# zfwangDP/X2-GNN

Measured on AMD Instinct MI355X. Metric: molecules/sec (fwd+bwd) on QM9 U0, batch=128, 1/2/4/8 MI355X, higher is better.
Workload: dtype fp32; 1 GPU; xgnn_poly U0 train step (config.json: L=4, D=128, H=16, sbf 7x6), S160, fwd+loss+bwd+allreduce+clip+Adam+EMA; per_gpu_batch=128, global_batch=128, line_nodes_per_gpu=21058, triplets_per_gpu=194060, parallelism=dp1, hip_graph=True

## Files before the change

x2-gnn_amd/csrc/feature.hip:

```cpp
#include "common.hpp"

namespace x2g {
namespace {

typedef float f4 __attribute__((ext_vector_type(4)));

constexpr int kFN1 = 256;
constexpr int kFN2 = 128;
constexpr int kFKMax = 384;
constexpr int kFRows = 32;
constexpr int kFAS = kFKMax + 8;
constexpr int kFYS = kFN1 + 8;
constexpr int kFThreads = 512;

__device__ __forceinline__ f4 mfma4(float a, float b, f4 acc) {
  return __builtin_amdgcn_mfma_f32_16x16x4f32(a, b, acc, 0, 0, 0);
}
__device__ __forceinline__ float sigmoid_(float z) {
  return __builtin_amdgcn_rcpf(1.0f + __builtin_amdgcn_exp2f(-1.4426950408889634f * z));
}
__device__ __forceinline__ float silu_(float z) { return z * sigmoid_(z); }
__device__ __forceinline__ float silu_grad_(float z) {
  const float s = sigmoid_(z);
  return s * (1.0f + z * (1.0f - s));
}
__device__ __forceinline__ f4 zero4() { return f4{0.f, 0.f, 0.f, 0.f}; }

__device__ __forceinline__ f4 quad_t(f4 v, int j) {
  f4 b, c;
#pragma unroll
  for (int k = 0; k < 4; ++k) {
    const float t = dpp_mov<0xB1>(v[k ^ 1]);
    b[k] = ((k ^ j) & 1) ? t : v[k];
  }
#pragma unroll
  for (int k = 0; k < 4; ++k) {
    const float t = dpp_mov<0x4E>(b[k ^ 2]);
    c[k] = ((k ^ j) & 2) ? t : b[k];
  }
  return c;
}

__device__ __forceinline__ int64_t tpos(int64_t tf, int64_t tile16, int f, int g) {
  return (f >> 7) * tf + tile16 * 2048 + (f & 127) * 16 + 4 * g;
}

struct FeatFwdArgs {
  const float* x;
  const float* env;
  const float* w1;
  const float* b1;
  const float* w2;
  const float* b2;
  float* y2;
  float* xs_t;
  float* z1_t;
  float* y1_t;
  float* z2_t;
  int64_t R;
  int64_t tf;
  int K;
  int want_t;
};

__device__ __forceinline__ f4 w1_frag(const float* __restrict__ w1, int K, int c, int q, int g) {
  const int k = 16 * q + 4 * g;
  const int k0 = k < K ? k : K - 2, k1 = k + 2 < K ? k + 2 : K - 2;
  const float2 lo = *reinterpret_cast<const float2*>(w1 + c * K + k0);
  const float2 hi = *reinterpret_cast<const float2*>(w1 + c * K + k1);
  const float m0 = k < K ? 1.0f : 0.0f, m1 = k + 2 < K ? 1.0f : 0.0f;
  return f4{lo.x * m0, lo.y * m0, hi.x * m1, hi.y * m1};
}

constexpr int kFX4 = (kFRows * kFKMax / 4 + kFThreads - 1) / kFThreads;

struct XTile {
  f4 v[kFX4];
  float env;
};

__device__ __forceinline__ void xtile_load(const FeatFwdArgs& a, int64_t tile, XTile& t) {
  const int64_t r0 = tile * kFRows;
  const int64_t R = a.R;
  const int nr = R - r0 < kFRows ? static_cast<int>(R - r0) : kFRows;
  const float* src = a.x + r0 * a.K;
  const int n = nr * a.K;
#pragma unroll
  for (int u = 0; u < kFX4; ++u) {
    const int q = threadIdx.x + kFThreads * u;
    if (4 * q + 3 < n) {
      t.v[u] = *reinterpret_cast<const f4*>(src + 4 * q);
    } else {
#pragma unroll
      for (int e = 0; e < 4; ++e) t.v[u][e] = 4 * q + e < n ? src[4 * q + e] : 0.0f;
    }
  }
  const int r = threadIdx.x;
  t.env = (r < nr && a.env) ? a.env[r0 + r] : 1.0f;
}

__global__ void __launch_bounds__(kFThreads, 1) feat_fwd_kernel(const FeatFwdArgs a) {
  __shared__ __attribute__((aligned(16))) float A[kFRows * kFAS];
  __shared__ __attribute__((aligned(16))) float Y1[kFRows * kFYS];
  __shared__ float envs[kFRows];
  const int tid = threadIdx.x, lane = tid & 63, w = tid >> 6;
  const int i = lane & 15, g = lane >> 4;
  const int K = a.K, KQ = (K + 15) / 16;
  const float invK = 1.0f / static_cast<float>(K);
  const int64_t R = a.R;
  const float* w2s = a.w2 + (16 * w + i) * kFN1 + 4 * g;
  const float b2v = a.b2 ? a.b2[16 * w + i] : 0.0f;
  const int c1a = 32 * w + i, c1b = c1a + 16;
  const float b1a = a.b1 ? a.b1[c1a] : 0.0f, b1b = a.b1 ? a.b1[c1b] : 0.0f;
  for (int idx = tid; idx < kFRows * (kFKMax - K); idx += kFThreads) {
    const int r = idx / (kFKMax - K), c = K + idx % (kFKMax - K);
    A[r * kFAS + c] = 0.0f;
  }
  const int64_t ntiles = (R + kFRows - 1) / kFRows;
  XTile xt;
  if (static_cast<int64_t>(blockIdx.x) < ntiles) xtile_load(a, blockIdx.x, xt);
  for (int64_t tile = blockIdx.x; tile < ntiles; tile += gridDim.x) {
    const int64_t r0 = tile * kFRows;
    const int nr = R - r0 < kFRows ? static_cast<int>(R - r0) : kFRows;
    __syncthreads();
    {
      const int n = nr * K;
#pragma unroll
      for (int u = 0; u < kFX4; ++u) {
        const int q = tid + kFThreads * u;
#pragma unroll
        for (int e = 0; e < 4; ++e) {
          const int j = 4 * q + e;
          if (j < kFRows * K) {
            int r = static_cast<int>(static_cast<float>(j) * invK);
            r -= r * K > j ? 1 : 0;
            r += (r + 1) * K <= j ? 1 : 0;
            A[r * kFAS + (j - r * K)] = j < n ? xt.v[u][e] : 0.0f;
          }
        }
      }
      if (tid < kFRows) envs[tid] = xt.env;
    }
    __syncthreads();
    f4 wa0 = w1_frag(a.w1, K, c1a, 0, g), wb0 = w1_frag(a.w1, K, c1b, 0, g);
    f4 wa1 = w1_frag(a.w1, K, c1a, 1, g), wb1 = w1_frag(a.w1, K, c1b, 1, g);
    if (tile + gridDim.x < ntiles) xtile_load(a, tile + gridDim.x, xt);
    auto xs_store = [&](int it) {
      const int rt = it / 3, p = it % 3;
      const int64_t t16 = r0 / 16 + rt;
      if (!a.want_t || t16 * 16 >= R || 128 * p >= K) return;
      const int f = tid >> 2, rr = 16 * rt + 4 * (tid & 3);
      f4 v;
#pragma unroll
      for (int e = 0; e < 4; ++e) v[e] = A[(rr + e) * kFAS + 128 * p + f] * envs[rr + e];
      *reinterpret_cast<f4*>(a.xs_t + p * a.tf + t16 * 2048 + 4 * tid) = v;
    };
    f4 acc[2][2] = {{zero4(), zero4()}, {zero4(), zero4()}};
    const int KQn = KQ;
    f4 a0 = *reinterpret_cast<const f4*>(A + i * kFAS + 4 * g);
    f4 a1 = *reinterpret_cast<const f4*>(A + (16 + i) * kFAS + 4 * g);
    auto group = [&](int q, f4& ba, f4& bb) {
      const int qa = q + 1 < KQn ? q + 1 : q;
      const f4 n0 = *reinterpret_cast<const f4*>(A + i * kFAS + 16 * qa + 4 * g);
      const f4 n1 = *reinterpret_cast<const f4*>(A + (16 + i) * kFAS + 16 * qa + 4 * g);
#pragma unroll
      for (int e = 0; e < 4; ++e) {
        acc[0][0] = mfma4(a0[e], ba[e], acc[0][0]);
        acc[0][1] = mfma4(a0[e], bb[e], acc[0][1]);
        acc[1][0] = mfma4(a1[e], ba[e], acc[1][0]);
        acc[1][1] = mfma4(a1[e], bb[e], acc[1][1]);
      }
      const int qb = q + 2 < KQn ? q + 2 : q;
      ba = w1_frag(a.w1, K, c1a, qb, g);
      bb = w1_frag(a.w1, K, c1b, qb, g);
      a0 = n0;
      a1 = n1;
    };
    for (int q = 0; q < KQn; q += 2) {
      group(q, wa0, wb0);
      if (q + 1 < KQn) group(q + 1, wa1, wb1);
    }
    f4 wq[3];
    wq[0] = *reinterpret_cast<const f4*>(w2s);
    wq[1] = *reinterpret_cast<const f4*>(w2s + 16);
#pragma unroll
    for (int rb = 0; rb < 2; ++rb) {
      const int64_t t16 = r0 / 16 + rb;
      const bool tile_ok = t16 * 16 < R;
#pragma unroll
      for (int cb = 0; cb < 2; ++cb) {
        const int c = cb ? c1b : c1a;
        const float bias = cb ? b1b : b1a;
        f4 z, y;
#pragma unroll
        for (int e = 0; e < 4; ++e) {
          const int r = 16 * rb + 4 * g + e;
          const bool ok = r < nr;
          z[e] = ok ? fmaf(acc[rb][cb][e], envs[r], bias) : 0.0f;
          y[e] = ok ? silu_(z[e]) : 0.0f;
          Y1[r * kFYS + c] = y[e];
        }
        if (tile_ok && a.want_t) {
          *reinterpret_cast<f4*>(a.z1_t + tpos(a.tf, t16, c, g)) = z;
          *reinterpret_cast<f4*>(a.y1_t + tpos(a.tf, t16, c, g)) = y;
        }
      }
    }
    __syncthreads();
    f4 acc2[2] = {zero4(), zero4()};
    {
      f4 y0 = *reinterpret_cast<const f4*>(Y1 + i * kFYS + 4 * g);
      f4 y1 = *reinterpret_cast<const f4*>(Y1 + (16 + i) * kFYS + 4 * g);
#pragma unroll
      for (int q = 0; q < 16; ++q) {
        const int qa = q + 1 < 16 ? q + 1 : q;
        const f4 n0 = *reinterpret_cast<const f4*>(Y1 + i * kFYS + 16 * qa + 4 * g);
        const f4 n1 = *reinterpret_cast<const f4*>(Y1 + (16 + i) * kFYS + 16 * qa + 4 * g);
        if (q + 2 < 16) wq[(q + 2) % 3] = *reinterpret_cast<const f4*>(w2s + 16 * (q + 2));
        __builtin_amdgcn_sched_barrier(0);
#pragma unroll
        for (int e = 0; e < 4; ++e) {
          acc2[0] = mfma4(y0[e], wq[q % 3][e], acc2[0]);
          acc2[1] = mfma4(y1[e], wq[q % 3][e], acc2[1]);
        }
        y0 = n0;
        y1 = n1;
      }
    }
    const int c2 = 16 * w + i;
    const int qj = i & 3, qm = i >> 2;
#pragma unroll
    for (int rb = 0; rb < 2; ++rb) {
      const int64_t t16 = r0 / 16 + rb;
      if (t16 * 16 >= R) continue;
      f4 z, y;
#pragma unroll
      for (int e = 0; e < 4; ++e) {
        const int r = 16 * rb + 4 * g + e;
        z[e] = r < nr ? acc2[rb][e] + b2v : 0.0f;
        y[e] = silu_(z[e]);
      }
      const f4 yt = quad_t(y, qj);
      const int ry = 16 * rb + 4 * g + qj;
      if (ry < nr) *reinterpret_cast<f4*>(a.y2 + (r0 + ry) * kFN2 + 16 * w + 4 * qm) = yt;
      if (a.want_t) *reinterpret_cast<f4*>(a.z2_t + tpos(a.tf, t16, c2, g)) = z;
    }
    for (int it = 0; it < 6; ++it) xs_store(it);
  }
}

struct FeatBwdArgs {
  const float* dy;
  const float* z2_t;
  const float* z1_t;
  const float* w2;
  float* dz2_t;
  float* dz1_t;
  int64_t R;
  int64_t tf;
};

constexpr int kFDS = kFN2 + 8;

__global__ void __launch_bounds__(kFThreads, 1) feat_bwd_kernel(const FeatBwdArgs a) {
  __shared__ __attribute__((aligned(16))) float DZ[kFRows * kFDS];
  const int tid = threadIdx.x, lane = tid & 63, w = tid >> 6;
  const int i = lane & 15, g = lane >> 4;
  const int64_t R = a.R;
  const int ca = 32 * w + i, cb = ca + 16;
  f4 wa[8], wb[8];
#pragma unroll
  for (int q = 0; q < 8; ++q)
#pragma unroll
    for (int e = 0; e < 4; ++e) {
      wa[q][e] = a.w2[(16 * q + 4 * g + e) * kFN1 + ca];
      wb[q][e] = a.w2[(16 * q + 4 * g + e) * kFN1 + cb];
    }
  const int c2 = 16 * w + i;
  const int64_t ntiles = (R + kFRows - 1) / kFRows;
  struct In {
    f4 z2[2];
    float dy[2][4];
  };
  auto load_in = [&](int64_t tile, In& in) {
    const int64_t r0 = tile * kFRows;
    const int nr = R - r0 < kFRows ? static_cast<int>(R - r0) : kFRows;
#pragma unroll
    for (int rb = 0; rb < 2; ++rb) {
      const int64_t t16 = r0 / 16 + rb;
      in.z2[rb] = t16 * 16 < R ? *reinterpret_cast<const f4*>(a.z2_t + tpos(a.tf, t16, c2, g)) : zero4();
#pragma unroll
      for (int e = 0; e < 4; ++e) {
        const int r = 16 * rb + 4 * g + e;
        in.dy[rb][e] = r < nr ? a.dy[(r0 + r) * kFN2 + c2] : 0.0f;
      }
    }
  };
  In cur;
  if (static_cast<int64_t>(blockIdx.x) < ntiles) load_in(blockIdx.x, cur);
  for (int64_t tile = blockIdx.x; tile < ntiles; tile += gridDim.x) {
    const int64_t r0 = tile * kFRows;
    const int nr = R - r0 < kFRows ? static_cast<int>(R - r0) : kFRows;
    __syncthreads();
#pragma unroll
    for (int rb = 0; rb < 2; ++rb) {
      const int64_t t16 = r0 / 16 + rb;
      const bool tile_ok = t16 * 16 < R;
      f4 d;
#pragma unroll
      for (int e = 0; e < 4; ++e) {
        const int r = 16 * rb + 4 * g + e;
        d[e] = r < nr ? cur.dy[rb][e] * silu_grad_(cur.z2[rb][e]) : 0.0f;
        DZ[r * kFDS + c2] = d[e];
      }
      if (tile_ok) *reinterpret_cast<f4*>(a.dz2_t + tpos(a.tf, t16, c2, g)) = d;
    }
    f4 z1v[2][2];
#pragma unroll
    for (int rb = 0; rb < 2; ++rb) {
      const int64_t t16 = r0 / 16 + rb;
      const int64_t tt = t16 * 16 < R ? t16 : r0 / 16;
#pragma unroll
      for (int k = 0; k < 2; ++k) z1v[rb][k] = *reinterpret_cast<const f4*>(a.z1_t + tpos(a.tf, tt, k ? cb : ca, g));
    }
    if (tile + gridDim.x < ntiles) load_in(tile + gridDim.x, cur);
    __syncthreads();
    f4 acc[2][2] = {{zero4(), zero4()}, {zero4(), zero4()}};
#pragma unroll
    for (int q = 0; q < 8; ++q) {
      const f4 a0 = *reinterpret_cast<const f4*>(DZ + i * kFDS + 16 * q + 4 * g);
      const f4 a1 = *reinterpret_cast<const f4*>(DZ + (16 + i) * kFDS + 16 * q + 4 * g);
#pragma unroll
      for (int e = 0; e < 4; ++e) {
        acc[0][0] = mfma4(a0[e], wa[q][e], acc[0][0]);
        acc[0][1] = mfma4(a0[e], wb[q][e], acc[0][1]);
        acc[1][0] = mfma4(a1[e], wa[q][e], acc[1][0]);
        acc[1][1] = mfma4(a1[e], wb[q][e], acc[1][1]);
      }
    }
#pragma unroll
    for (int rb = 0; rb < 2; ++rb) {
      const int64_t t16 = r0 / 16 + rb;
      if (t16 * 16 >= R) continue;
#pragma unroll
      for (int k = 0; k < 2; ++k) {
        const int c = k ? cb : ca;
        f4 d;
#pragma unroll
        for (int e = 0; e < 4; ++e) d[e] = acc[rb][k][e] * silu_grad_(z1v[rb][k][e]);
        *reinterpret_cast<f4*>(a.dz1_t + tpos(a.tf, t16, c, g)) = d;
      }
    }
  }
}

inline bool al16(const void* p) { return reinterpret_cast<uintptr_t>(p) % 16 == 0; }

inline unsigned feat_grid(int64_t R) {
  const int64_t tiles = (R + kFRows - 1) / kFRows;
  return static_cast<unsigned>(tiles < 256 ? tiles : 256);
}

}
}

using namespace x2g;

X2G_API int x2g_feat_fwd(const float* x, const float* env, int64_t rows, int32_t in_dim, const float* w1,
                         const float* b1, const float* w2, const float* b2, float* y, float* xs_t, float* z1_t,
                         float* y1_t, float* z2_t, void* stream) {
  if (rows < 0 || in_dim <= 0) return X2G_EINVAL;
  if (in_dim > kFKMax || in_dim % 2 || in_dim <= 2 * 128 || rows * kFKMax * 4 >= (int64_t(1) << 31))
    return X2G_EUNSUPPORTED;
  if (rows == 0) return X2G_OK;
  if (!x || !w1 || !w2 || !y) return X2G_EINVAL;
  const int nt = (xs_t != nullptr) + (z1_t != nullptr) + (y1_t != nullptr) + (z2_t != nullptr);
  if (nt != 0 && nt != 4) return X2G_EINVAL;
  if (!al16(x) || !al16(w2) || !al16(xs_t) || !al16(z1_t) || !al16(y1_t) || !al16(z2_t) ||
      reinterpret_cast<uintptr_t>(w1) % 8)
    return X2G_EUNSUPPORTED;
  FeatFwdArgs a{x, env, w1, b1, w2, b2, y, xs_t, z1_t, y1_t, z2_t, rows, x2g_chain_t_floats(rows, 128), in_dim,
                nt == 4 ? 1 : 0};
  feat_fwd_kernel<<<feat_grid(rows), kFThreads, 0, as_stream(stream)>>>(a);
  return last_launch_status();
}

X2G_API int x2g_feat_bwd(const float* dy, const float* z2_t, const float* z1_t, const float* w2, int64_t rows,
                         float* dz2_t, float* dz1_t, void* stream) {
  if (rows < 0) return X2G_EINVAL;
  if (rows * kFKMax * 4 >= (int64_t(1) << 31)) return X2G_EUNSUPPORTED;
  if (rows == 0) return X2G_OK;
  if (!dy || !z2_t || !z1_t || !w2 || !dz2_t || !dz1_t) return X2G_EINVAL;
  if (!al16(z2_t) || !al16(z1_t) || !al16(dz2_t) || !al16(dz1_t)) return X2G_EUNSUPPORTED;
  FeatBwdArgs a{dy, z2_t, z1_t, w2, dz2_t, dz1_t, rows, x2g_chain_t_floats(rows, 128)};
  feat_bwd_kernel<<<feat_grid(rows), kFThreads, 0, as_stream(stream)>>>(a);
  return last_launch_status();
}
```

x2-gnn_amd/csrc/rbf_gate.hip:

```cpp
#include "common.hpp"

namespace x2g {

constexpr int kGateRMax = 8;
constexpr int kGateBwdSplits = 128;

typedef float f4v __attribute__((ext_vector_type(4)));

template <int D>
__device__ __forceinline__ void stage_gate_weights(const float* __restrict__ W, const float* __restrict__ B, int R,
                                                   float* __restrict__ sw) {
  for (int i = threadIdx.x; i < D * R; i += blockDim.x) sw[i] = W[i];
  for (int i = threadIdx.x; i < D; i += blockDim.x) sw[D * kGateRMax + i] = B ? B[i] : 0.f;
  __syncthreads();
}

template <int LPR>
struct GateW {
  float w[4][kGateRMax];
  float b[4];
  __device__ __forceinline__ void load(const float* __restrict__ sw, int R, int sub) {
    constexpr int D = 4 * LPR;
#pragma unroll
    for (int i = 0; i < 4; ++i) {
      const int c = 4 * sub + i;
#pragma unroll
      for (int j = 0; j < kGateRMax; ++j) w[i][j] = j < R ? sw[c * R + j] : 0.f;
      b[i] = sw[D * kGateRMax + c];
    }
  }
  __device__ __forceinline__ f4v filter(const float (&rb)[kGateRMax]) const {
    f4v f;
#pragma unroll
    for (int i = 0; i < 4; ++i) {
      float a = b[i];
#pragma unroll
      for (int j = 0; j < kGateRMax; ++j) a = fmaf(w[i][j], rb[j], a);
      f[i] = a;
    }
    return f;
  }
};

__device__ __forceinline__ void load_rbf(const float* __restrict__ rbf, int64_t r, int R, float (&rb)[kGateRMax]) {
#pragma unroll
  for (int j = 0; j < kGateRMax; ++j) rb[j] = rbf[r * R + (j < R ? j : R - 1)];
}

template <int LPR>
__global__ void __launch_bounds__(256) rbf_gate_fwd_kernel(const f4v* __restrict__ x, const float* __restrict__ rbf,
                                                           const float* __restrict__ W, const float* __restrict__ B,
                                                           int64_t rows, int R, f4v* __restrict__ out) {
  constexpr int RPB = 256 / LPR;
  constexpr int UNROLL = 4;
  __shared__ float sw[4 * LPR * (kGateRMax + 1)];
  stage_gate_weights<4 * LPR>(W, B, R, sw);
  const int sub = threadIdx.x % LPR, slot = threadIdx.x / LPR;
  GateW<LPR> gw;
  gw.load(sw, R, sub);
  const int64_t stride = static_cast<int64_t>(gridDim.x) * RPB * UNROLL;
  for (int64_t r0 = static_cast<int64_t>(blockIdx.x) * RPB * UNROLL + slot; r0 < rows; r0 += stride) {
    float rb[UNROLL][kGateRMax];
    f4v xv[UNROLL];
#pragma unroll
    for (int u = 0; u < UNROLL; ++u) {
      const int64_t r = r0 + u * RPB, rc = r < rows ? r : rows - 1;
      load_rbf(rbf, rc, R, rb[u]);
      xv[u] = x[rc * LPR + sub];
    }
#pragma unroll
    for (int u = 0; u < UNROLL; ++u) {
      const int64_t r = r0 + u * RPB;
      if (r < rows) out[r * LPR + sub] = xv[u] * gw.filter(rb[u]);
    }
  }
}

constexpr int kGateMaxJobs = X2G_GATE_MAX_JOBS;
struct PoolJobs {
  const f4v* x[kGateMaxJobs];
  const float* w[kGateMaxJobs];
  const float* b[kGateMaxJobs];
  f4v* out[kGateMaxJobs];
};

template <int LPR>
__global__ void __launch_bounds__(256) rbf_pool_fwd_kernel(const PoolJobs J, const float* __restrict__ rbf,
                                                           const int32_t* __restrict__ rowptr, int64_t G, int R) {
  constexpr int RPI = 64 / LPR;
  constexpr int UNROLL = 8;
  __shared__ float sw[4 * LPR * (kGateRMax + 1)];
  const int job = blockIdx.y;
  const f4v* __restrict__ x = J.x[job];
  f4v* __restrict__ out = J.out[job];
  stage_gate_weights<4 * LPR>(J.w[job], J.b[job], R, sw);
  const int lane = threadIdx.x & 63;
  const int sub = lane % LPR, slot = lane / LPR;
  GateW<LPR> gw;
  gw.load(sw, R, sub);
  const int nwaves = gridDim.x * 4;
  const int jl = (lane & 15) < R ? (lane & 15) : R - 1;
  for (int64_t g = uniform(blockIdx.x * 4 + (threadIdx.x >> 6)); g < G; g += nwaves) {
    const int r0 = uniform(rowptr[g]), r1 = uniform(rowptr[g + 1]);
    f4v acc = {0.f, 0.f, 0.f, 0.f};
    for (int rb0 = r0; rb0 < r1; rb0 += UNROLL * RPI) {
      f4v v[UNROLL];
      float rv[UNROLL];
#pragma unroll
      for (int u = 0; u < UNROLL; ++u) {
        const int r = rb0 + u * RPI + slot;
        const int rc = r < r1 ? r : r1 - 1;
        v[u] = x[static_cast<int64_t>(rc) * LPR + sub];
        rv[u] = rbf[static_cast<int64_t>(rc) * R + jl];
      }
#pragma unroll
      for (int u = 0; u < UNROLL; ++u) {
        const float ok = rb0 + u * RPI + slot < r1 ? 1.f : 0.f;
        float rb[kGateRMax];
        rb[0] = dpp_mov<0x150>(rv[u]);
        rb[1] = dpp_mov<0x151>(rv[u]);
        rb[2] = dpp_mov<0x152>(rv[u]);
        rb[3] = dpp_mov<0x153>(rv[u]);
        rb[4] = dpp_mov<0x154>(rv[u]);
        rb[5] = dpp_mov<0x155>(rv[u]);
        rb[6] = dpp_mov<0x156>(rv[u]);
        rb[7] = dpp_mov<0x157>(rv[u]);
        acc += (v[u] * gw.filter(rb)) * ok;
      }
    }
#pragma unroll
    for (int off = LPR; off < 64; off <<= 1) {
#pragma unroll
      for (int i = 0; i < 4; ++i) acc[i] += __shfl_xor(acc[i], off, kWave);
    }
    if (slot == 0) out[g * LPR + sub] = acc;
  }
}

template <int LPR>
__device__ __forceinline__ float transpose_sum(const float (&p)[kGateRMax], int sub, int& j) {
  constexpr int o1 = LPR / 2, o2 = LPR / 4, o3 = LPR / 8;
  const bool h1 = sub & o1, h2 = sub & o2, h3 = sub & o3;
  float q[4], r[2];
#pragma unroll
  for (int k = 0; k < 4; ++k) {
    const float send = h1 ? p[k] : p[k + 4];
    const float recv = xor_xchg<o1>(send);
    q[k] = (h1 ? p[k + 4] : p[k]) + recv;
  }
#pragma unroll
  for (int k = 0; k < 2; ++k) {
    const float send = h2 ? q[k] : q[k + 2];
    const float recv = xor_xchg<o2>(send);
    r[k] = (h2 ? q[k + 2] : q[k]) + recv;
  }
  float t;
  {
    const float send = h3 ? r[0] : r[1];
    const float recv = xor_xchg<o3>(send);
    t = (h3 ? r[1] : r[0]) + recv;
  }
  if constexpr (o3 >= 8) t += xor_xchg<4>(t);
  if constexpr (o3 >= 4) t += xor_xchg<2>(t);
  if constexpr (o3 >= 2) t += xor_xchg<1>(t);
  j = 4 * h1 + 2 * h2 + h3;
  return t;
}

struct GateBwdJobs {
  const f4v* g[kGateMaxJobs];
  const f4v* x[kGateMaxJobs];
  const float* w[kGateMaxJobs];
  const float* b[kGateMaxJobs];
  f4v* dx[kGateMaxJobs];
  const f4v* dx_add[kGateMaxJobs];
  float* drbf[kGateMaxJobs];
  float* part_w[kGateMaxJobs];
  float* part_b[kGateMaxJobs];
};

template <int LPR>
__global__ void __launch_bounds__(256) rbf_gate_bwd_kernel(const GateBwdJobs J, const int32_t* __restrict__ owner,
                                                           const float* __restrict__ rbf, int64_t rows, int R,
                                                           int drbf_acc) {
  constexpr int RPB = 256 / LPR;
  constexpr int D = 4 * LPR;
  __shared__ float red[RPB * D * (kGateRMax + 1)];
  __shared__ float sw[D * (kGateRMax + 1)];
  const int job = blockIdx.y;
  const f4v* __restrict__ g = J.g[job];
  const f4v* __restrict__ x = J.x[job];
  f4v* __restrict__ dx = J.dx[job];
  const f4v* __restrict__ dx_add = J.dx_add[job];
  float* __restrict__ drbf = J.drbf[job];
  float* __restrict__ part_w = J.part_w[job];
  float* __restrict__ part_b = J.part_b[job];
  stage_gate_weights<D>(J.w[job], J.b[job], R, sw);
  const int sub = threadIdx.x % LPR, slot = threadIdx.x / LPR;
  GateW<LPR> gw;
  gw.load(sw, R, sub);
  float aw[4][kGateRMax], ab[4];
#pragma unroll
  for (int i = 0; i < 4; ++i) {
    ab[i] = 0.f;
#pragma unroll
    for (int j = 0; j < kGateRMax; ++j) aw[i][j] = 0.f;
  }
  constexpr int UNROLL = 3;
  const int jd = 4 * ((sub & (LPR / 2)) != 0) + 2 * ((sub & (LPR / 4)) != 0) + ((sub & (LPR / 8)) != 0);
  const bool acc_drbf = drbf && drbf_acc && jd < R;
  const int64_t per = (rows + gridDim.x - 1) / gridDim.x;
  const int64_t lo = per * blockIdx.x, hi = lo + per < rows ? lo + per : rows;
  const int jl = (threadIdx.x & 15) < R ? (threadIdx.x & 15) : R - 1;
  auto desc = [](const void* p, int64_t bytes) {
    return __builtin_amdgcn_make_buffer_rsrc(const_cast<void*>(p), static_cast<short>(0),
                                             static_cast<int>(bytes < 0x7fffffff ? bytes : 0x7fffffff), 0x00020000);
  };
  const __amdgpu_buffer_rsrc_t own_r = desc(owner, owner ? rows * 4 : 0);
  const __amdgpu_buffer_rsrc_t od_r = desc(drbf, (drbf && drbf_acc) ? rows * R * 4 : 0);
  const __amdgpu_buffer_rsrc_t add_r = desc(dx_add, dx_add ? rows * LPR * 16 : 0);
  const bool has_owner = owner != nullptr;
  for (int64_t r0 = lo + slot; r0 < hi; r0 += RPB * UNROLL) {
    float rv[UNROLL];
    f4v gv[UNROLL], xv[UNROLL], av[UNROLL];
    float od[UNROLL];
#pragma unroll
    for (int u = 0; u < UNROLL; ++u) {
      const int64_t r = r0 + u * RPB, rc = r < hi ? r : hi - 1;
      rv[u] = rbf[rc * R + jl];
      od[u] = __builtin_bit_cast(float, __builtin_amdgcn_raw_buffer_load_b32(
                                            od_r, acc_drbf ? static_cast<int>((rc * R + jd) * 4) : 0x7ffffff0, 0, 0));
      const int ow = static_cast<int>(__builtin_amdgcn_raw_buffer_load_b32(own_r, static_cast<int>(rc * 4), 0, 0));
      const int64_t o = has_owner ? ow : rc;
      gv[u] = g[o * LPR + sub];
      xv[u] = x[rc * LPR + sub];
      av[u] = __builtin_bit_cast(f4v, __builtin_amdgcn_raw_buffer_load_b128(
                                         add_r, static_cast<int>((rc * LPR + sub) * 16), 0, 0));
    }
#pragma unroll
    for (int u = 0; u < UNROLL; ++u) {
      const int64_t r = r0 + u * RPB;
      const bool ok = r < hi;
      const float m = ok ? 1.f : 0.f;
      float rb[kGateRMax];
      rb[0] = dpp_mov<0x150>(rv[u]);
      rb[1] = dpp_mov<0x151>(rv[u]);
      rb[2] = dpp_mov<0x152>(rv[u]);
      rb[3] = dpp_mov<0x153>(rv[u]);
      rb[4] = dpp_mov<0x154>(rv[u]);
      rb[5] = dpp_mov<0x155>(rv[u]);
      rb[6] = dpp_mov<0x156>(rv[u]);
      rb[7] = dpp_mov<0x157>(rv[u]);
      if (dx && ok) {
        f4v d = gv[u] * gw.filter(rb);
        if (dx_add) d += av[u];
        dx[r * LPR + sub] = d;
      }
      const f4v df = gv[u] * xv[u] * m;
#pragma unroll
      for (int i = 0; i < 4; ++i) {
        ab[i] += df[i];
#pragma unroll
        for (int j = 0; j < kGateRMax; ++j) aw[i][j] = fmaf(df[i], rb[j], aw[i][j]);
      }
      if (drbf) {
        float p[kGateRMax];
#pragma unroll
        for (int j = 0; j < kGateRMax; ++j) {
          float a = 0.f;
#pragma unroll
          for (int i = 0; i < 4; ++i) a = fmaf(df[i], gw.w[i][j], a);
          p[j] = a;
        }
        int j;
        const float tot = transpose_sum<LPR>(p, sub, j);
        if ((sub & (LPR / 8 - 1)) == 0 && ok && j < R) drbf[r * R + j] = tot + od[u];
      }
    }
  }
  const int per_slot = D * (R + 1);
  float* mine = red + slot * per_slot;
#pragma unroll
  for (int i = 0; i < 4; ++i) {
    const int c = 4 * sub + i;
    for (int j = 0; j < R; ++j) mine[c * R + j] = aw[i][j];
    mine[D * R + c] = ab[i];
  }
  __syncthreads();
  for (int idx = threadIdx.x; idx < per_slot; idx += 256) {
    float s = 0.f;
    for (int sl = 0; sl < RPB; ++sl) s += red[sl * per_slot + idx];
    if (idx < D * R)
      part_w[static_cast<int64_t>(blockIdx.x) * D * R + idx] = s;
    else if (part_b)
      part_b[static_cast<int64_t>(blockIdx.x) * D + idx - D * R] = s;
  }
}

inline bool gate_shape_ok(int D, int R) { return R >= 1 && R <= kGateRMax && (D == 64 || D == 128 || D == 256); }

inline int gate_bwd_splits(int64_t rows) {
  const int64_t want = (rows + 7) / 8;
  return static_cast<int>(want < kGateBwdSplits ? (want < 1 ? 1 : want) : kGateBwdSplits);
}

}

using namespace x2g;

static inline bool al16(const void* p) { return reinterpret_cast<uintptr_t>(p) % 16 == 0; }

X2G_API int x2g_rbf_gate_fwd(const float* x, const float* rbf, const float* w, const float* b, int64_t rows, int32_t D,
                             int32_t R, float* out, void* stream) {
  if (rows < 0 || !gate_shape_ok(D, R)) return rows < 0 ? X2G_EINVAL : X2G_EUNSUPPORTED;
  if (rows == 0) return X2G_OK;
  if (!x || !rbf || !w || !out) return X2G_EINVAL;
  if (!al16(x) || !al16(out)) return X2G_EINVAL;
  const auto* xv = reinterpret_cast<const f4v*>(x);
  auto* ov = reinterpret_cast<f4v*>(out);
  const int64_t want = (rows * D / 4 + 1023) / 1024;
  const unsigned grid = static_cast<unsigned>(want < 2048 ? want : 2048);
  hipStream_t st = as_stream(stream);
  switch (D) {
    case 64: rbf_gate_fwd_kernel<16><<<grid, 256, 0, st>>>(xv, rbf, w, b, rows, R, ov); break;
    case 128: rbf_gate_fwd_kernel<32><<<grid, 256, 0, st>>>(xv, rbf, w, b, rows, R, ov); break;
    default: rbf_gate_fwd_kernel<64><<<grid, 256, 0, st>>>(xv, rbf, w, b, rows, R, ov); break;
  }
  return last_launch_status();
}

static int pool_launch(const PoolJobs& J, int n_jobs, const float* rbf, const int32_t* rowptr, int64_t G, int D, int R,
                       hipStream_t st) {
  const int64_t want = (G + 3) / 4;
  const dim3 grid(static_cast<unsigned>(want < 2048 ? want : 2048), static_cast<unsigned>(n_jobs));
  switch (D) {
    case 64: rbf_pool_fwd_kernel<16><<<grid, 256, 0, st>>>(J, rbf, rowptr, G, R); break;
    case 128: rbf_pool_fwd_kernel<32><<<grid, 256, 0, st>>>(J, rbf, rowptr, G, R); break;
    default: rbf_pool_fwd_kernel<64><<<grid, 256, 0, st>>>(J, rbf, rowptr, G, R); break;
  }
  return last_launch_status();
}

X2G_API int x2g_rbf_pool_fwd(const float* x, const float* rbf, const float* w, const float* b, const int32_t* rowptr,
                             int64_t G, int32_t D, int32_t R, float* out, void* stream) {
  if (G < 0 || !gate_shape_ok(D, R)) return G < 0 ? X2G_EINVAL : X2G_EUNSUPPORTED;
  if (G == 0) return X2G_OK;
  if (!x || !rbf || !w || !rowptr || !out) return X2G_EINVAL;
  if (!al16(x) || !al16(out)) return X2G_EINVAL;
  PoolJobs J{};
  J.x[0] = reinterpret_cast<const f4v*>(x);
  J.w[0] = w;
  J.b[0] = b;
  J.out[0] = reinterpret_cast<f4v*>(out);
  return pool_launch(J, 1, rbf, rowptr, G, D, R, as_stream(stream));
}

X2G_API int x2g_rbf_pool_fwd_batch(const x2g_gate_job* jobs, int32_t n_jobs, const float* rbf, const int32_t* rowptr,
                                   int64_t G, int32_t D, int32_t R, void* stream) {
  if (!jobs || n_jobs < 1 || n_jobs > kGateMaxJobs || G < 0) return X2G_EINVAL;
  if (!gate_shape_ok(D, R)) return X2G_EUNSUPPORTED;
  if (G == 0) return X2G_OK;
  if (!rbf || !rowptr) return X2G_EINVAL;
  PoolJobs J{};
  for (int j = 0; j < n_jobs; ++j) {
    const x2g_gate_job& q = jobs[j];
    if (!q.x || !q.w || !q.out) return X2G_EINVAL;
    if (!al16(q.x) || !al16(q.out)) return X2G_EINVAL;
    J.x[j] = reinterpret_cast<const f4v*>(q.x);
    J.w[j] = q.w;
    J.b[j] = q.b;
    J.out[j] = reinterpret_cast<f4v*>(q.out);
  }
  return pool_launch(J, n_jobs, rbf, rowptr, G, D, R, as_stream(stream));
}

static int gate_bwd_launch(const GateBwdJobs& J, int n_jobs, const int32_t* owner, const float* rbf, int64_t rows,
                           int D, int R, int drbf_acc, int splits, hipStream_t st) {
  constexpr int64_t kLim = int64_t(1) << 31;
  bool add = false;
  for (int j = 0; j < n_jobs; ++j) add = add || J.dx_add[j] != nullptr;
  if ((owner && rows * 4 >= kLim) || (drbf_acc && rows * static_cast<int64_t>(R) * 4 >= kLim) ||
      (add && rows * static_cast<int64_t>(D) * 4 >= kLim))
    return X2G_EUNSUPPORTED;
  const dim3 grid(static_cast<unsigned>(splits), static_cast<unsigned>(n_jobs));
  switch (D) {
    case 64: rbf_gate_bwd_kernel<16><<<grid, 256, 0, st>>>(J, owner, rbf, rows, R, drbf_acc); break;
    case 128: rbf_gate_bwd_kernel<32><<<grid, 256, 0, st>>>(J, owner, rbf, rows, R, drbf_acc); break;
    default: rbf_gate_bwd_kernel<64><<<grid, 256, 0, st>>>(J, owner, rbf, rows, R, drbf_acc); break;
  }
  return last_launch_status();
}

X2G_API int32_t x2g_rbf_gate_bwd_splits(int64_t rows) { return rows > 0 ? gate_bwd_splits(rows) : 0; }

X2G_API size_t x2g_rbf_gate_bwd_workspace(int64_t rows, int32_t D, int32_t R) {
  if (rows <= 0 || D <= 0 || R <= 0) return 0;
  return static_cast<size_t>(gate_bwd_splits(rows)) * D * (R + 1) * sizeof(float);
}

X2G_API int x2g_rbf_gate_bwd(const float* g, const int32_t* owner, const float* x, const float* rbf, const float* w,
                             const float* b, int64_t rows, int32_t D, int32_t R, float* dx, const float* dx_add,
                             float* drbf, float* dw, float* db, int flags, void* ws, size_t wsb, void* stream) {
  if (rows < 0 || !dw) return X2G_EINVAL;
  if (!gate_shape_ok(D, R)) return X2G_EUNSUPPORTED;
  if (dx_add && !dx) return X2G_EINVAL;
  if (flags & ~(X2G_ACCUM_WGRAD | X2G_DEFER_SLAB_SUM | X2G_GATE_DRBF_ACCUM)) return X2G_EINVAL;
  const bool accum = flags & X2G_ACCUM_WGRAD;
  const int drbf_acc = (flags & X2G_GATE_DRBF_ACCUM) ? 1 : 0;
  hipStream_t st = as_stream(stream);
  if (rows == 0) {
    if (flags & X2G_DEFER_SLAB_SUM) return X2G_EINVAL;
    if (accum) return X2G_OK;
    hipError_t e = hipMemsetAsync(dw, 0, sizeof(float) * D * R, st);
    if (e == hipSuccess && db) e = hipMemsetAsync(db, 0, sizeof(float) * D, st);
    return e == hipSuccess ? X2G_OK : static_cast<int>(e);
  }
  if (!g || !x || !rbf || !w) return X2G_EINVAL;
// ... 68 lines not shown
```

Baseline: 59090 molecules/s.

## Enlarge feature MLP row tiles and software-pipeline RBF pooling loads

The forward feature MLP kernel now processes 48-row tiles (three 16-row blocks) over contiguous per-block ranges instead of 32-row tiles strided across the grid, reusing each w1/w2 fragment across more MFMA row blocks. The backward kernel keeps a separate 32-row tile size. The RBF pooling kernel double-buffers segment loads, prefetching the next batch and the next segments' row pointers while consuming the current one, and its grid is capped at a few waves per SIMD. The aim is to cut weight-load overhead and hide global-memory latency, at the cost of more registers, extra template instantiations, and possible load imbalance.

```diff
diff --git a/x2-gnn_amd/csrc/feature.hip b/x2-gnn_amd/csrc/feature.hip
--- a/x2-gnn_amd/csrc/feature.hip
+++ b/x2-gnn_amd/csrc/feature.hip
@@ -8,7 +8,9 @@
 constexpr int kFN1 = 256;
 constexpr int kFN2 = 128;
 constexpr int kFKMax = 384;
-constexpr int kFRows = 32;
+constexpr int kFBlk = 3;
+constexpr int kFRows = 16 * kFBlk;
+constexpr int kFBRows = 32;
 constexpr int kFAS = kFKMax + 8;
 constexpr int kFYS = kFN1 + 8;
 constexpr int kFThreads = 512;
@@ -72,21 +74,21 @@
   return f4{lo.x * m0, lo.y * m0, hi.x * m1, hi.y * m1};
 }
 
-constexpr int kFX4 = (kFRows * kFKMax / 4 + kFThreads - 1) / kFThreads;
-
+constexpr int kFX4Max = (kFRows * kFKMax / 4 + kFThreads - 1) / kFThreads;
+constexpr int kFX4 = kFX4Max - 1;
+
+template <int NX4>
 struct XTile {
-  f4 v[kFX4];
+  f4 v[NX4];
   float env;
 };
 
-__device__ __forceinline__ void xtile_load(const FeatFwdArgs& a, int64_t tile, XTile& t) {
-  const int64_t r0 = tile * kFRows;
-  const int64_t R = a.R;
-  const int nr = R - r0 < kFRows ? static_cast<int>(R - r0) : kFRows;
+template <int NX4>
+__device__ __forceinline__ void xtile_load(const FeatFwdArgs& a, int64_t r0, int nr, XTile<NX4>& t) {
   const float* src = a.x + r0 * a.K;
   const int n = nr * a.K;
 #pragma unroll
-  for (int u = 0; u < kFX4; ++u) {
+  for (int u = 0; u < NX4; ++u) {
     const int q = threadIdx.x + kFThreads * u;
     if (4 * q + 3 < n) {
       t.v[u] = *reinterpret_cast<const f4*>(src + 4 * q);
@@ -99,6 +101,12 @@
   t.env = (r < nr && a.env) ? a.env[r0 + r] : 1.0f;
 }
 
+template <int NB>
+struct FeatBlocks {
+  static constexpr int value = NB;
+};
+
+template <int NX4>
 __global__ void __launch_bounds__(kFThreads, 1) feat_fwd_kernel(const FeatFwdArgs a) {
   __shared__ __attribute__((aligned(16))) float A[kFRows * kFAS];
   __shared__ __attribute__((aligned(16))) float Y1[kFRows * kFYS];
@@ -116,136 +124,165 @@
     const int r = idx / (kFKMax - K), c = K + idx % (kFKMax - K);
     A[r * kFAS + c] = 0.0f;
   }
-  const int64_t ntiles = (R + kFRows - 1) / kFRows;
-  XTile xt;
-  if (static_cast<int64_t>(blockIdx.x) < ntiles) xtile_load(a, blockIdx.x, xt);
-  for (int64_t tile = blockIdx.x; tile < ntiles; tile += gridDim.x) {
-    const int64_t r0 = tile * kFRows;
-    const int nr = R - r0 < kFRows ? static_cast<int>(R - r0) : kFRows;
-    __syncthreads();
-    {
-      const int n = nr * K;
-#pragma unroll
-      for (int u = 0; u < kFX4; ++u) {
-        const int q = tid + kFThreads * u;
-#pragma unroll
-        for (int e = 0; e < 4; ++e) {
-          const int j = 4 * q + e;
-          if (j < kFRows * K) {
-            int r = static_cast<int>(static_cast<float>(j) * invK);
-            r -= r * K > j ? 1 : 0;
-            r += (r + 1) * K <= j ? 1 : 0;
-            A[r * kFAS + (j - r * K)] = j < n ? xt.v[u][e] : 0.0f;
+  const int64_t nblk = (R + 15) / 16;
+  const int64_t blk0 = blockIdx.x * nblk / gridDim.x, blk1 = (blockIdx.x + 1) * nblk / gridDim.x;
+  auto tile_blocks = [&](int64_t tb) { return blk1 - tb < kFBlk ? static_cast<int>(blk1 - tb) : kFBlk; };
+  auto tile_rows = [&](int64_t tb, int nbt) {
+    return R - tb * 16 < 16 * nbt ? static_cast<int>(R - tb * 16) : 16 * nbt;
+  };
+  XTile<NX4> xt;
+  if (blk0 < blk1) xtile_load(a, blk0 * 16, tile_rows(blk0, tile_blocks(blk0)), xt);
+  for (int64_t tb = blk0; tb < blk1; tb += kFBlk) {
+    const int64_t r0 = tb * 16;
+    const int nbt = tile_blocks(tb);
+    const int nr = tile_rows(tb, nbt);
+    auto body = [&](auto nbc) {
+      constexpr int NB = decltype(nbc)::value;
+      __syncthreads();
+      {
+        const int n = nr * K;
+#pragma unroll
+        for (int u = 0; u < NX4; ++u) {
+          int q = tid + kFThreads * u;
+          if (NX4 > kFX4) asm volatile("" : "+v"(q));
+          if (16 * NB * kFKMax <= 4 * kFThreads * u) continue;
+#pragma unroll
+          for (int e = 0; e < 4; ++e) {
+            const int j = 4 * q + e;
+            if (j < 16 * NB * K) {
+              int r = static_cast<int>(static_cast<float>(j) * invK);
+              r -= r * K > j ? 1 : 0;
+              r += (r + 1) * K <= j ? 1 : 0;
+              A[r * kFAS + (j - r * K)] = j < n ? xt.v[u][e] : 0.0f;
+            }
           }
         }
-      }
-      if (tid < kFRows) envs[tid] = xt.env;
-    }
-    __syncthreads();
-    f4 wa0 = w1_frag(a.w1, K, c1a, 0, g), wb0 = w1_frag(a.w1, K, c1b, 0, g);
-    f4 wa1 = w1_frag(a.w1, K, c1a, 1, g), wb1 = w1_frag(a.w1, K, c1b, 1, g);
-    if (tile + gridDim.x < ntiles) xtile_load(a, tile + gridDim.x, xt);
-    auto xs_store = [&](int it) {
-      const int rt = it / 3, p = it % 3;
-      const int64_t t16 = r0 / 16 + rt;
-      if (!a.want_t || t16 * 16 >= R || 128 * p >= K) return;
-      const int f = tid >> 2, rr = 16 * rt + 4 * (tid & 3);
-      f4 v;
-#pragma unroll
-      for (int e = 0; e < 4; ++e) v[e] = A[(rr + e) * kFAS + 128 * p + f] * envs[rr + e];
-      *reinterpret_cast<f4*>(a.xs_t + p * a.tf + t16 * 2048 + 4 * tid) = v;
-    };
-    f4 acc[2][2] = {{zero4(), zero4()}, {zero4(), zero4()}};
-    const int KQn = KQ;
-    f4 a0 = *reinterpret_cast<const f4*>(A + i * kFAS + 4 * g);
-    f4 a1 = *reinterpret_cast<const f4*>(A + (16 + i) * kFAS + 4 * g);
-    auto group = [&](int q, f4& ba, f4& bb) {
-      const int qa = q + 1 < KQn ? q + 1 : q;
-      const f4 n0 = *reinterpret_cast<const f4*>(A + i * kFAS + 16 * qa + 4 * g);
-      const f4 n1 = *reinterpret_cast<const f4*>(A + (16 + i) * kFAS + 16 * qa + 4 * g);
-#pragma unroll
-      for (int e = 0; e < 4; ++e) {
-        acc[0][0] = mfma4(a0[e], ba[e], acc[0][0]);
-        acc[0][1] = mfma4(a0[e], bb[e], acc[0][1]);
-        acc[1][0] = mfma4(a1[e], ba[e], acc[1][0]);
-        acc[1][1] = mfma4(a1[e], bb[e], acc[1][1]);
-      }
-      const int qb = q + 2 < KQn ? q + 2 : q;
-      ba = w1_frag(a.w1, K, c1a, qb, g);
-      bb = w1_frag(a.w1, K, c1b, qb, g);
-      a0 = n0;
-      a1 = n1;
-    };
-    for (int q = 0; q < KQn; q += 2) {
-      group(q, wa0, wb0);
-      if (q + 1 < KQn) group(q + 1, wa1, wb1);
-    }
-    f4 wq[3];
-    wq[0] = *reinterpret_cast<const f4*>(w2s);
-    wq[1] = *reinterpret_cast<const f4*>(w2s + 16);
-#pragma unroll
-    for (int rb = 0; rb < 2; ++rb) {
-      const int64_t t16 = r0 / 16 + rb;
-      const bool tile_ok = t16 * 16 < R;
-#pragma unroll
-      for (int cb = 0; cb < 2; ++cb) {
-        const int c = cb ? c1b : c1a;
-        const float bias = cb ? b1b : b1a;
+        if (tid < 16 * NB) envs[tid] = xt.env;
+      }
+      __syncthreads();
+      f4 wa0 = w1_frag(a.w1, K, c1a, 0, g), wb0 = w1_frag(a.w1, K, c1b, 0, g);
+      f4 wa1 = w1_frag(a.w1, K, c1a, 1, g), wb1 = w1_frag(a.w1, K, c1b, 1, g);
+      if (tb + kFBlk < blk1) {
+        const int64_t tn = tb + kFBlk;
+        xtile_load(a, tn * 16, tile_rows(tn, tile_blocks(tn)), xt);
+      }
+      auto xs_store = [&](int it) {
+        const int rt = it / 3, p = it % 3;
+        const int64_t t16 = tb + rt;
+        if (!a.want_t || rt >= nbt || 128 * p >= K) return;
+        const int f = tid >> 2, rr = 16 * rt + 4 * (tid & 3);
+        f4 v;
+#pragma unroll
+        for (int e = 0; e < 4; ++e) v[e] = A[(rr + e) * kFAS + 128 * p + f] * envs[rr + e];
+        *reinterpret_cast<f4*>(a.xs_t + p * a.tf + t16 * 2048 + 4 * tid) = v;
+      };
+      f4 acc[NB][2];
+#pragma unroll
+      for (int rb = 0; rb < NB; ++rb) acc[rb][0] = acc[rb][1] = zero4();
+      const int KQn = KQ;
+      f4 ar[NB];
+#pragma unroll
+      for (int rb = 0; rb < NB; ++rb) ar[rb] = *reinterpret_cast<const f4*>(A + (16 * rb + i) * kFAS + 4 * g);
+      auto group = [&](int q, f4& ba, f4& bb) {
+        const int qa = q + 1 < KQn ? q + 1 : q;
+        f4 nx[NB];
+#pragma unroll
+        for (int rb = 0; rb < NB; ++rb)
+          nx[rb] = *reinterpret_cast<const f4*>(A + (16 * rb + i) * kFAS + 16 * qa + 4 * g);
+#pragma unroll
+        for (int e = 0; e < 4; ++e) {
+#pragma unroll
+          for (int rb = 0; rb < NB; ++rb) {
+            acc[rb][0] = mfma4(ar[rb][e], ba[e], acc[rb][0]);
+            acc[rb][1] = mfma4(ar[rb][e], bb[e], acc[rb][1]);
+          }
+        }
+        const int qb = q + 2 < KQn ? q + 2 : q;
+        ba = w1_frag(a.w1, K, c1a, qb, g);
+        bb = w1_frag(a.w1, K, c1b, qb, g);
+#pragma unroll
+        for (int rb = 0; rb < NB; ++rb) ar[rb] = nx[rb];
+      };
+      for (int q = 0; q < KQn; q += 2) {
+        group(q, wa0, wb0);
+        if (q + 1 < KQn) group(q + 1, wa1, wb1);
+      }
+      f4 wq[3];
+      wq[0] = *reinterpret_cast<const f4*>(w2s);
+      wq[1] = *reinterpret_cast<const f4*>(w2s + 16);
+#pragma unroll
+      for (int rb = 0; rb < NB; ++rb) {
+        const int64_t t16 = tb + rb;
+        const bool tile_ok = rb < nbt;
+#pragma unroll
+        for (int cb = 0; cb < 2; ++cb) {
+          const int c = cb ? c1b : c1a;
+          const float bias = cb ? b1b : b1a;
+          f4 z, y;
+#pragma unroll
+          for (int e = 0; e < 4; ++e) {
+            const int r = 16 * rb + 4 * g + e;
+            const bool ok = r < nr;
+            z[e] = ok ? fmaf(acc[rb][cb][e], envs[r], bias) : 0.0f;
+            y[e] = ok ? silu_(z[e]) : 0.0f;
+            Y1[r * kFYS + c] = y[e];
+          }
+          if (tile_ok && a.want_t) {
+            *reinterpret_cast<f4*>(a.z1_t + tpos(a.tf, t16, c, g)) = z;
+            *reinterpret_cast<f4*>(a.y1_t + tpos(a.tf, t16, c, g)) = y;
+          }
+        }
+      }
+      __syncthreads();
+      f4 acc2[NB];
+#pragma unroll
+      for (int rb = 0; rb < NB; ++rb) acc2[rb] = zero4();
+      {
+        f4 yr[NB];
+#pragma unroll
+        for (int rb = 0; rb < NB; ++rb) yr[rb] = *reinterpret_cast<const f4*>(Y1 + (16 * rb + i) * kFYS + 4 * g);
+#pragma unroll
+        for (int q = 0; q < 16; ++q) {
+          const int qa = q + 1 < 16 ? q + 1 : q;
+          f4 nx[NB];
+#pragma unroll
+          for (int rb = 0; rb < NB; ++rb)
+            nx[rb] = *reinterpret_cast<const f4*>(Y1 + (16 * rb + i) * kFYS + 16 * qa + 4 * g);
+          if (q + 2 < 16) wq[(q + 2) % 3] = *reinterpret_cast<const f4*>(w2s + 16 * (q + 2));
+          __builtin_amdgcn_sched_barrier(0);
+#pragma unroll
+          for (int e = 0; e < 4; ++e) {
+#pragma unroll
+            for (int rb = 0; rb < NB; ++rb) acc2[rb] = mfma4(yr[rb][e], wq[q % 3][e], acc2[rb]);
+          }
+#pragma unroll
+          for (int rb = 0; rb < NB; ++rb) yr[rb] = nx[rb];
+        }
+      }
+      const int c2 = 16 * w + i;
+      const int qj = i & 3, qm = i >> 2;
+#pragma unroll
+      for (int rb = 0; rb < NB; ++rb) {
+        const int64_t t16 = tb + rb;
+        if (rb >= nbt) continue;
         f4 z, y;
 #pragma unroll
         for (int e = 0; e < 4; ++e) {
           const int r = 16 * rb + 4 * g + e;
-          const bool ok = r < nr;
-          z[e] = ok ? fmaf(acc[rb][cb][e], envs[r], bias) : 0.0f;
-          y[e] = ok ? silu_(z[e]) : 0.0f;
-          Y1[r * kFYS + c] = y[e];
+          z[e] = r < nr ? acc2[rb][e] + b2v : 0.0f;
+          y[e] = silu_(z[e]);
         }
-        if (tile_ok && a.want_t) {
-          *reinterpret_cast<f4*>(a.z1_t + tpos(a.tf, t16, c, g)) = z;
-          *reinterpret_cast<f4*>(a.y1_t + tpos(a.tf, t16, c, g)) = y;
-        }
-      }
-    }
-    __syncthreads();
-    f4 acc2[2] = {zero4(), zero4()};
-    {
-      f4 y0 = *reinterpret_cast<const f4*>(Y1 + i * kFYS + 4 * g);
-      f4 y1 = *reinterpret_cast<const f4*>(Y1 + (16 + i) * kFYS + 4 * g);
-#pragma unroll
-      for (int q = 0; q < 16; ++q) {
-        const int qa = q + 1 < 16 ? q + 1 : q;
-        const f4 n0 = *reinterpret_cast<const f4*>(Y1 + i * kFYS + 16 * qa + 4 * g);
-        const f4 n1 = *reinterpret_cast<const f4*>(Y1 + (16 + i) * kFYS + 16 * qa + 4 * g);
-        if (q + 2 < 16) wq[(q + 2) % 3] = *reinterpret_cast<const f4*>(w2s + 16 * (q + 2));
-        __builtin_amdgcn_sched_barrier(0);
-#pragma unroll
-        for (int e = 0; e < 4; ++e) {
-          acc2[0] = mfma4(y0[e], wq[q % 3][e], acc2[0]);
-          acc2[1] = mfma4(y1[e], wq[q % 3][e], acc2[1]);
-        }
-        y0 = n0;
-        y1 = n1;
-      }
-    }
-    const int c2 = 16 * w + i;
-    const int qj = i & 3, qm = i >> 2;
-#pragma unroll
-    for (int rb = 0; rb < 2; ++rb) {
-      const int64_t t16 = r0 / 16 + rb;
-      if (t16 * 16 >= R) continue;
-      f4 z, y;
-#pragma unroll
-      for (int e = 0; e < 4; ++e) {
-        const int r = 16 * rb + 4 * g + e;
-        z[e] = r < nr ? acc2[rb][e] + b2v : 0.0f;
-        y[e] = silu_(z[e]);
-      }
-      const f4 yt = quad_t(y, qj);
-      const int ry = 16 * rb + 4 * g + qj;
-      if (ry < nr) *reinterpret_cast<f4*>(a.y2 + (r0 + ry) * kFN2 + 16 * w + 4 * qm) = yt;
-      if (a.want_t) *reinterpret_cast<f4*>(a.z2_t + tpos(a.tf, t16, c2, g)) = z;
-    }
-    for (int it = 0; it < 6; ++it) xs_store(it);
+        const f4 yt = quad_t(y, qj);
+        const int ry = 16 * rb + 4 * g + qj;
+        if (ry < nr) *reinterpret_cast<f4*>(a.y2 + (r0 + ry) * kFN2 + 16 * w + 4 * qm) = yt;
+        if (a.want_t) *reinterpret_cast<f4*>(a.z2_t + tpos(a.tf, t16, c2, g)) = z;
+      }
+      for (int it = 0; it < 3 * NB; ++it) xs_store(it);
+    };
+    if (nbt == kFBlk)
+      body(FeatBlocks<kFBlk>{});
+    else
+      body(FeatBlocks<2>{});
   }
 }
 
@@ -263,7 +300,7 @@
 constexpr int kFDS = kFN2 + 8;
 
 __global__ void __launch_bounds__(kFThreads, 1) feat_bwd_kernel(const FeatBwdArgs a) {
-  __shared__ __attribute__((aligned(16))) float DZ[kFRows * kFDS];
+  __shared__ __attribute__((aligned(16))) float DZ[kFBRows * kFDS];
   const int tid = threadIdx.x, lane = tid & 63, w = tid >> 6;
   const int i = lane & 15, g = lane >> 4;
   const int64_t R = a.R;
@@ -277,14 +314,14 @@
       wb[q][e] = a.w2[(16 * q + 4 * g + e) * kFN1 + cb];
     }
   const int c2 = 16 * w + i;
-  const int64_t ntiles = (R + kFRows - 1) / kFRows;
+  const int64_t ntiles = (R + kFBRows - 1) / kFBRows;
   struct In {
     f4 z2[2];
     float dy[2][4];
   };
   auto load_in = [&](int64_t tile, In& in) {
-    const int64_t r0 = tile * kFRows;
-    const int nr = R - r0 < kFRows ? static_cast<int>(R - r0) : kFRows;
+    const int64_t r0 = tile * kFBRows;
+    const int nr = R - r0 < kFBRows ? static_cast<int>(R - r0) : kFBRows;
 #pragma unroll
     for (int rb = 0; rb < 2; ++rb) {
       const int64_t t16 = r0 / 16 + rb;
@@ -299,8 +336,8 @@
   In cur;
   if (static_cast<int64_t>(blockIdx.x) < ntiles) load_in(blockIdx.x, cur);
   for (int64_t tile = blockIdx.x; tile < ntiles; tile += gridDim.x) {
-    const int64_t r0 = tile * kFRows;
-    const int nr = R - r0 < kFRows ? static_cast<int>(R - r0) : kFRows;
+    const int64_t r0 = tile * kFBRows;
+    const int nr = R - r0 < kFBRows ? static_cast<int>(R - r0) : kFBRows;
     __syncthreads();
 #pragma unroll
     for (int rb = 0; rb < 2; ++rb) {
@@ -356,9 +393,14 @@
 
 inline bool al16(const void* p) { return reinterpret_cast<uintptr_t>(p) % 16 == 0; }
 
-inline unsigned feat_grid(int64_t R) {
-  const int64_t tiles = (R + kFRows - 1) / kFRows;
+inline unsigned feat_bwd_grid(int64_t R) {
+  const int64_t tiles = (R + kFBRows - 1) / kFBRows;
   return static_cast<unsigned>(tiles < 256 ? tiles : 256);
+}
+
+inline unsigned feat_fwd_grid(int64_t R) {
+  const int64_t want = ((R + 15) / 16 + 1) / 2;
+  return static_cast<unsigned>(want < 256 ? want : 256);
 }
 
 }
@@ -381,7 +423,10 @@
     return X2G_EUNSUPPORTED;
   FeatFwdArgs a{x, env, w1, b1, w2, b2, y, xs_t, z1_t, y1_t, z2_t, rows, x2g_chain_t_floats(rows, 128), in_dim,
                 nt == 4 ? 1 : 0};
-  feat_fwd_kernel<<<feat_grid(rows), kFThreads, 0, as_stream(stream)>>>(a);
+  if (kFRows * in_dim <= 4 * kFThreads * kFX4)
+    feat_fwd_kernel<kFX4><<<feat_fwd_grid(rows), kFThreads, 0, as_stream(stream)>>>(a);
+  else
+    feat_fwd_kernel<kFX4Max><<<feat_fwd_grid(rows), kFThreads, 0, as_stream(stream)>>>(a);
   return last_launch_status();
 }
 
@@ -393,6 +438,6 @@
   if (!dy || !z2_t || !z1_t || !w2 || !dz2_t || !dz1_t) return X2G_EINVAL;
   if (!al16(z2_t) || !al16(z1_t) || !al16(dz2_t) || !al16(dz1_t)) return X2G_EUNSUPPORTED;
   FeatBwdArgs a{dy, z2_t, z1_t, w2, dz2_t, dz1_t, rows, x2g_chain_t_floats(rows, 128)};
-  feat_bwd_kernel<<<feat_grid(rows), kFThreads, 0, as_stream(stream)>>>(a);
+  feat_bwd_kernel<<<feat_bwd_grid(rows), kFThreads, 0, as_stream(stream)>>>(a);
   return last_launch_status();
 }
diff --git a/x2-gnn_amd/csrc/rbf_gate.hip b/x2-gnn_amd/csrc/rbf_gate.hip
--- a/x2-gnn_amd/csrc/rbf_gate.hip
+++ b/x2-gnn_amd/csrc/rbf_gate.hip
@@ -89,51 +89,97 @@
                                                            const int32_t* __restrict__ rowptr, int64_t G, int R) {
   constexpr int RPI = 64 / LPR;
   constexpr int UNROLL = 8;
+  constexpr int STEP = UNROLL * RPI;
   __shared__ float sw[4 * LPR * (kGateRMax + 1)];
   const int job = blockIdx.y;
   const f4v* __restrict__ x = J.x[job];
   f4v* __restrict__ out = J.out[job];
-  stage_gate_weights<4 * LPR>(J.w[job], J.b[job], R, sw);
   const int lane = threadIdx.x & 63;
   const int sub = lane % LPR, slot = lane / LPR;
+  const int nwaves = gridDim.x * 4;
+  const int jl = (lane & 15) < R ? (lane & 15) : R - 1;
+  const int64_t g0 = uniform(blockIdx.x * 4 + (threadIdx.x >> 6));
+  const int nrows = uniform(rowptr[G]);
+  struct Batch {
+    f4v v[UNROLL];
+    float rv[UNROLL];
+  };
+  auto load_batch = [&](int rb0, int r1, Batch& b) {
+#pragma unroll
+    for (int u = 0; u < UNROLL; ++u) {
+      const int r = rb0 + u * RPI + slot;
+      int rc = r < r1 ? r : r1 - 1;
+      rc = rc < 0 ? 0 : rc;
+      b.v[u] = x[static_cast<int64_t>(rc) * LPR + sub];
+      b.rv[u] = rbf[static_cast<int64_t>(rc) * R + jl];
+    }
+  };
+  auto seg_rows = [&](int64_t g, int at, int& r0, int& r1) {
+    r0 = r1 = at;
+    if (g < G) {
+      r0 = uniform(rowptr[g]);
+      r1 = uniform(rowptr[g + 1]);
+    }
+  };
+  int c0, c1, n0, n1;
+  Batch ba, bb;
+  seg_rows(g0, 0, c0, c1);
+  if (nrows > 0) load_batch(c0, c1, ba);
+  seg_rows(g0 + nwaves, c1, n0, n1);
+  stage_gate_weights<4 * LPR>(J.w[job], J.b[job], R, sw);
   GateW<LPR> gw;
   gw.load(sw, R, sub);
-  const int nwaves = gridDim.x * 4;
-  const int jl = (lane & 15) < R ? (lane & 15) : R - 1;
-  for (int64_t g = uniform(blockIdx.x * 4 + (threadIdx.x >> 6)); g < G; g += nwaves) {
-    const int r0 = uniform(rowptr[g]), r1 = uniform(rowptr[g + 1]);
-    f4v acc = {0.f, 0.f, 0.f, 0.f};
-    for (int rb0 = r0; rb0 < r1; rb0 += UNROLL * RPI) {
-      f4v v[UNROLL];
-      float rv[UNROLL];
-#pragma unroll
-      for (int u = 0; u < UNROLL; ++u) {
-        const int r = rb0 + u * RPI + slot;
-        const int rc = r < r1 ? r : r1 - 1;
-        v[u] = x[static_cast<int64_t>(rc) * LPR + sub];
-        rv[u] = rbf[static_cast<int64_t>(rc) * R + jl];
+  if (nrows <= 0) {
+    for (int64_t g = g0; g < G; g += nwaves)
+      if (slot == 0) out[g * LPR + sub] = f4v{0.f, 0.f, 0.f, 0.f};
+    return;
+  }
+  auto consume = [&](const Batch& b, int rb0, int r1, f4v& acc) {
+#pragma unroll
+    for (int u = 0; u < UNROLL; ++u) {
+      if (rb0 + u * RPI >= r1) continue;
+      const float ok = rb0 + u * RPI + slot < r1 ? 1.f : 0.f;
+      float rb[kGateRMax];
+      rb[0] = dpp_mov<0x150>(b.rv[u]);
+      rb[1] = dpp_mov<0x151>(b.rv[u]);
+      rb[2] = dpp_mov<0x152>(b.rv[u]);
+      rb[3] = dpp_mov<0x153>(b.rv[u]);
+      rb[4] = dpp_mov<0x154>(b.rv[u]);
+      rb[5] = dpp_mov<0x155>(b.rv[u]);
+      rb[6] = dpp_mov<0x156>(b.rv[u]);
+      rb[7] = dpp_mov<0x157>(b.rv[u]);
+      acc += (b.v[u] * gw.filter(rb)) * ok;
+    }
+  };
+  int64_t g = g0;
+  int rb0 = c0, m0, m1;
+  seg_rows(g0 + 2 * static_cast<int64_t>(nwaves), n1, m0, m1);
+  f4v acc = {0.f, 0.f, 0.f, 0.f};
+  auto step = [&](Batch& cur, Batch& nxt) {
+    const bool last = rb0 + STEP >= c1;
+    load_batch(last ? n0 : rb0 + STEP, last ? n1 : c1, nxt);
+    if (rb0 < c1) consume(cur, rb0, c1, acc);
+    if (last) {
+#pragma unroll
+      for (int off = LPR; off < 64; off <<= 1) {
+#pragma unroll
+        for (int i = 0; i < 4; ++i) acc[i] += __shfl_xor(acc[i], off, kWave);
       }
-#pragma unroll
-      for (int u = 0; u < UNROLL; ++u) {
-        const float ok = rb0 + u * RPI + slot < r1 ? 1.f : 0.f;
-        float rb[kGateRMax];
-        rb[0] = dpp_mov<0x150>(rv[u]);
-        rb[1] = dpp_mov<0x151>(rv[u]);
-        rb[2] = dpp_mov<0x152>(rv[u]);
-        rb[3] = dpp_mov<0x153>(rv[u]);
-        rb[4] = dpp_mov<0x154>(rv[u]);
-        rb[5] = dpp_mov<0x155>(rv[u]);
-        rb[6] = dpp_mov<0x156>(rv[u]);
-        rb[7] = dpp_mov<0x157>(rv[u]);
-        acc += (v[u] * gw.filter(rb)) * ok;
-      }
-    }
-#pragma unroll
-    for (int off = LPR; off < 64; off <<= 1) {
-#pragma unroll
-      for (int i = 0; i < 4; ++i) acc[i] += __shfl_xor(acc[i], off, kWave);
-    }
-    if (slot == 0) out[g * LPR + sub] = acc;
+      if (slot == 0) out[g * LPR + sub] = acc;
+      acc = f4v{0.f, 0.f, 0.f, 0.f};
+      g += nwaves;
+      c0 = n0, c1 = n1;
+      n0 = m0, n1 = m1;
+      rb0 = c0;
+      seg_rows(g + 2 * static_cast<int64_t>(nwaves), n1, m0, m1);
+    } else {
+      rb0 += STEP;
+    }
+  };
+  while (g < G) {
+    step(ba, bb);
+    if (g >= G) break;
+    step(bb, ba);
   }
 }
 
@@ -299,6 +345,13 @@
 
 inline bool gate_shape_ok(int D, int R) { return R >= 1 && R <= kGateRMax && (D == 64 || D == 128 || D == 256); }
 
+constexpr int kPoolWavesPerSimd = 2;
+inline unsigned pool_grid(int64_t G, int n_jobs) {
+  const int64_t cap = kPoolWavesPerSimd * 256 / n_jobs;
+  const int64_t want = (G + 3) / 4;
+  return static_cast<unsigned>(want < cap ? want : cap);
+}
+
 inline int gate_bwd_splits(int64_t rows) {
   const int64_t want = (rows + 7) / 8;
   return static_cast<int>(want < kGateBwdSplits ? (want < 1 ? 1 : want) : kGateBwdSplits);
@@ -331,8 +384,7 @@
 
 static int pool_launch(const PoolJobs& J, int n_jobs, const float* rbf, const int32_t* rowptr, int64_t G, int D, int R,
                        hipStream_t st) {
-  const int64_t want = (G + 3) / 4;
-  const dim3 grid(static_cast<unsigned>(want < 2048 ? want : 2048), static_cast<unsigned>(n_jobs));
+  const dim3 grid(pool_grid(G, n_jobs), static_cast<unsigned>(n_jobs));
   switch (D) {
     case 64: rbf_pool_fwd_kernel<16><<<grid, 256, 0, st>>>(J, rbf, rowptr, G, R); break;
     case 128: rbf_pool_fwd_kernel<32><<<grid, 256, 0, st>>>(J, rbf, rowptr, G, R); break;
```

Result: no change. 59370 molecules/s (median of 6 runs) (+0.5%).
